# themattrosen/Planeverb

Measured on AMD Instinct MI355X. Metric: grid_cell_updates_per_s, higher is better.
Workload: dtype f32

## Files before the change

include/planeverb_amd.h:

```cpp
#ifndef PLANEVERB_AMD_H
#define PLANEVERB_AMD_H

#include <stddef.h>
#include <stdint.h>

#ifdef __cplusplus
extern "C" {
#endif

#if defined(__GNUC__)
#define PVA_EXPORT __attribute__((visibility("default")))
#else
#define PVA_EXPORT
#endif


typedef struct PlaneverbOutput {
    float occlusion;
    float wetGain;
    float rt60;
    float lowpass;
    float directionX;
    float directionY;
    float sourceDirectionX;
// ... 209 lines not shown
#define PVA_SHAPE_CAPSULE 2
#define PVA_SHAPE_WALL_PATH 3
#define PVA_SHAPE_POLYGON 4
PVA_EXPORT int PvAmdHostRoundShapeCoverage(float gridSizeX, float gridSizeY, int gridResolution, int kind, const float* xy,
                                           int n, float radius, uint8_t* cover);

PVA_EXPORT int PvAmdRun(PvAmdSolver* s, float lx, float ly, float lz);
PVA_EXPORT int PvAmdRunAsync(PvAmdSolver* s, float lx, float ly, float lz);
PVA_EXPORT int PvAmdRunAsyncAfter(PvAmdSolver* s, PvAmdSolver* prev, float lx, float ly, float lz);
PVA_EXPORT int PvAmdSync(PvAmdSolver* s);
PVA_EXPORT int PvAmdRunBatch(PvAmdSolver* const* solvers, int n, const float* listenersXYZ, int wait);
PVA_EXPORT float PvAmdClockProbe(int device, float* byMemtimeMHz);
PVA_EXPORT int PvAmdBandwidthProbe(int device, float* gbPerS4);
PVA_EXPORT int PvAmdGetTimings(PvAmdSolver* s, PvAmdTimings* out);
PVA_EXPORT int PvAmdLastRunResidentWindow(PvAmdSolver* s);

PVA_EXPORT int PvAmdSetEmitters(PvAmdSolver* s, const float* xyz, int n);
PVA_EXPORT int PvAmdGetOutput(PvAmdSolver* s, float ex, float ey, float ez, PlaneverbOutput* out);
PVA_EXPORT int PvAmdSetOutputQueries(PvAmdSolver* s, const float* xyz, int n);
PVA_EXPORT int PvAmdGetQueriedOutputs(PvAmdSolver* s, PlaneverbOutput* out, int n);
PVA_EXPORT int PvAmdCopyResults(PvAmdSolver* s, float* res8, float* delay);
PVA_EXPORT int PvAmdCopyResultsBlock(PvAmdSolver* s, int r0, int c0, int nr, int nc, float* res8, float* delay);
PVA_EXPORT int PvAmdGetImpulseResponse(PvAmdSolver* s, int cx, int cy, float* out3T);
PVA_EXPORT int PvAmdGetImpulseResponseCells(PvAmdSolver* s, int cx, int cy, PlaneverbCell* outT);
PVA_EXPORT int PvAmdCopyFields(PvAmdSolver* s, float* pr, float* vx, float* vy);
PVA_EXPORT int PvAmdCopyHistoryPlane(PvAmdSolver* s, int t, float* pr);
typedef struct PvAmdRoomMetrics {
    float c50, c80, d50, ts, e50, l50, e80, l80, total, moment;
} PvAmdRoomMetrics;
PVA_EXPORT int PvAmdComputeRoomMetrics(PvAmdSolver* s, float* ms);
// ... 62 lines not shown
```

planeverb_amd/api.py:

```python
import ctypes as C
import os
from collections import namedtuple

import numpy as np

from .build import LIB_PATH

PV_INVALID_DRY_GAIN = -1.0
PV_INVALID_ID = -1

PVA_OPT_DENSE_HISTORY = 1
PVA_OPT_NUM_STEPS = 2
PVA_OPT_SKIP_ANALYSIS = 3
PVA_OPT_USE_GRAPH = 4
PVA_OPT_STEPS_PER_LAUNCH = 5
PVA_OPT_TILE_ROWS = 6
PVA_OPT_NO_FREE_GRID = 7
PVA_OPT_TIME_KERNELS = 8
PVA_OPT_TILE_ORDER = 9
PVA_OPT_SMALL_GRID_KERNEL = 10
PVA_OPT_PACKED_MATH = 11
PVA_OPT_STREAMING_ANALYSIS = 12
PVA_OPT_STREAM_ROWS = 13
PVA_OPT_MERGED_LAUNCH = 14
# ... 169 lines not shown
    "PvAmdHostEdgeLayerTablesR0": (C.c_int, [C.c_float, C.c_float, C.c_int, C.POINTER(C.c_int), C.c_double, _fp]),
    "PvAmdHostEdgeLayerTables": (C.c_int, [C.c_float, C.c_float, C.c_int, C.POINTER(C.c_int), _fp]),
    "PvAmdHostEnclosure": (C.c_int, [C.POINTER(C.c_ubyte)] + [C.c_int] * 7 + [C.POINTER(C.c_int)]),
    "PvAmdHostOrientedBoxVertices": (C.c_int, [C.c_float] * 6 + [_fp]),
    "PvAmdHostShape": (C.c_int, [_fp, C.c_int, C.c_float, _fp]),
    "PvAmdHostShapeCoverage": (C.c_int, [C.c_float, C.c_float, C.c_int, _fp, C.c_int, C.POINTER(C.c_ubyte)]),
    "PvAmdHostRoundShapeCoverage": (C.c_int, [C.c_float, C.c_float, C.c_int, C.c_int, _fp, C.c_int, C.c_float,
                                              C.POINTER(C.c_ubyte)]),
    "PvAmdRun": (C.c_int, [_vp] + [C.c_float] * 3),
    "PvAmdRunAsync": (C.c_int, [_vp] + [C.c_float] * 3),
    "PvAmdRunAsyncAfter": (C.c_int, [_vp, _vp] + [C.c_float] * 3),
    "PvAmdSync": (C.c_int, [_vp]),
    "PvAmdRunBatch": (C.c_int, [C.POINTER(_vp), C.c_int, _fp, C.c_int]),
    "PvAmdGetTimings": (C.c_int, [_vp, C.POINTER(PvAmdTimings)]),
    "PvAmdLastRunResidentWindow": (C.c_int, [_vp]),
    "PvAmdClockProbe": (C.c_float, [C.c_int, _fp]),
    "PvAmdBandwidthProbe": (C.c_int, [C.c_int, _fp]),
    "PvAmdSetEmitters": (C.c_int, [_vp, _fp, C.c_int]),
    "PvAmdGetOutput": (C.c_int, [_vp] + [C.c_float] * 3 + [C.POINTER(PlaneverbOutput)]),
    "PvAmdSetOutputQueries": (C.c_int, [_vp, _fp, C.c_int]),
    "PvAmdGetQueriedOutputs": (C.c_int, [_vp, C.POINTER(PlaneverbOutput), C.c_int]),
    "PvAmdCopyResults": (C.c_int, [_vp, _fp, _fp]),
    "PvAmdCopyResultsBlock": (C.c_int, [_vp, C.c_int, C.c_int, C.c_int, C.c_int, _fp, _fp]),
    "PvAmdGetImpulseResponse": (C.c_int, [_vp, C.c_int, C.c_int, _fp]),
    "PvAmdGetImpulseResponseCells": (C.c_int, [_vp, C.c_int, C.c_int, C.POINTER(PlaneverbCell)]),
    "PvAmdCopyFields": (C.c_int, [_vp, _fp, _fp, _fp]),
    "PvAmdCopyHistoryPlane": (C.c_int, [_vp, C.c_int, _fp]),
    "PvAmdComputeRoomMetrics": (C.c_int, [_vp, _fp]),
    "PvAmdCopyRoomMetrics": (C.c_int, [_vp, _fp]),
    "PvAmdCopyRoomMetricsBlock": (C.c_int, [_vp, C.c_int, C.c_int, C.c_int, C.c_int, _fp]),
# ... 847 lines not shown
    def run_async_after(self, prev, listener):
        _check(lib().PvAmdRunAsyncAfter(self._h, prev._h, *[float(v) for v in listener]))

    def sync(self):
        _check(lib().PvAmdSync(self._h))

    def run_steps(self, nsteps, with_pulse=False, listener=(0.0, 0.0, 0.0)):
        _check(lib().PvAmdRunSteps(self._h, int(nsteps), int(with_pulse), float(listener[0]), float(listener[2])))

    def last_run_resident_window(self):
        rc = lib().PvAmdLastRunResidentWindow(self._h)
        if rc < 0:
            raise PlaneverbError(last_error())
        return rc == 1

    def timings(self):
        t = PvAmdTimings()
        _check(lib().PvAmdGetTimings(self._h, t))
        return t

    def set_emitters(self, emitters):
        e = np.ascontiguousarray(emitters, np.float32).reshape(-1, 3)
        _check(lib().PvAmdSetEmitters(self._h, _f(e), len(e)))

    def get_output(self, emitter):
        o = PlaneverbOutput()
        _check(lib().PvAmdGetOutput(self._h, *[float(v) for v in emitter], o))
        return o

    def set_output_queries(self, emitters):
# ... 87 lines not shown
```

planeverb_amd/csrc/pv_analysis.hip:

```cpp
#include <hip/hip_runtime.h>

#include <cfloat>
#include <climits>
#include <cstdint>

#include "pv_analysis.h"
#include "pv_analysis_dev.h"
#include "pv_device.h"
#include "pv_launch.h"
#include "pv_libm.h"
#include "pv_prims.h"
namespace pva {



template <int CH>
__device__ __forceinline__ void rt60Chunk(const float (&pc)[CH], const int i0, const int startingPoint, float& edc,
                                          float& xysum, float& ysum) {
    float e[CH], y[CH];
#pragma unroll
    for (int k = 0; k < CH; ++k) {
        edc = (i0 - k >= startingPoint) ? edc + pc[k] * pc[k] : edc;
        e[k] = edc;
    }
// ... 15 lines not shown
    return *X < a.gx && *Y < a.gy;
}

#ifndef PV_ONSET_WAVES
#define PV_ONSET_WAVES 4
#endif
#ifndef PV_ONSET_SC
#define PV_ONSET_SC 32
#endif
constexpr int kOnsetWaves = PV_ONSET_WAVES, kOnsetSC = PV_ONSET_SC;
__global__ __launch_bounds__(64 * kOnsetWaves) void pv_onset_kernel(const AnalyzeArgs a) {
    __shared__ int found[64];
    if (analysisAborted(a)) return;
    const DynParams dyn = *a.dyn;
    const int lane = threadIdx.x & 63, wave = __builtin_amdgcn_readfirstlane((int)(threadIdx.x >> 6));
    const long long g = (long long)blockIdx.x * 64 + lane;
    const PlaneCell c = planeCell(a, dyn, g);
    const int T = a.T;
    int tF = INT_MAX;
    bool live = c.inGrid;
    if (live) {
        tF = a.tileFirst[c.tile];
        live = tF < T && a.coef[(size_t)(c.X + a.G) * a.pitch + (c.Y + a.G)].beta != 0.f;
    }
    const bool air = live;
    if (a.labels) {
        const int lX = dyn.lrow - a.G, lY = dyn.lcol - a.G;
        const int mine = live ? a.labels[(size_t)c.X * a.labelNY + c.Y] : -1;
        const int theirs = (lX >= 0 && lX <= a.gx && lY >= 0 && lY < a.labelNY) ? a.labels[(size_t)lX * a.labelNY + lY] : -2;
        live = live && mine == theirs;
    }
    if (wave == 0) found[lane] = INT_MAX;
    if (a.stamp && blockIdx.x == 0 && threadIdx.x == 0) a.stamp[1] = wall_clock64();
    __syncthreads();
    bool inPrev = false;
    if (a.box) {
        const int p0 = a.prevBox[0], p1 = a.prevBox[1], p2 = min(a.prevBox[2], a.gx - 1), p3 = min(a.prevBox[3], a.gy - 1);
        inPrev = c.inGrid && c.X >= p0 && c.X <= p2 && c.Y >= p1 && c.Y <= p3;
        if (p2 >= p0 && p3 >= p1) {
            const int wr0 = dyn.histRow0 - a.G, wc0 = dyn.histCol0 - a.G;
            const int wr1 = wr0 + min(a.winRows, a.gx - wr0) - 1, wc1 = wc0 + min(a.winCols, a.gy - wc0) - 1;
            if (p0 < wr0 || p2 > wr1 || p1 < wc0 || p3 > wc1)
                for (int r = p0 + (int)blockIdx.x; r <= p2; r += (int)gridDim.x)
                    for (int cc = p1 + (int)threadIdx.x; cc <= p3; cc += (int)blockDim.x)
                        if (r < wr0 || r > wr1 || cc < wc0 || cc > wc1) a.delay[r * a.gy + cc] = FLT_MAX;
        }
    }
    if (a.wholeWindow || a.box) {
        if (wave == 0 && c.inGrid && !live && (a.wholeWindow || inPrev)) a.delay[c.X * a.gy + c.Y] = FLT_MAX;
        if (blockIdx.x == 0 && wave == 1) {
            int n = 0;
            for (int i = lane; i < dyn.histTilesX * dyn.histTilesY; i += 64) {
                const int ti = dyn.histTileX0 + i / dyn.histTilesY, tj = dyn.histTileY0 + i % dyn.histTilesY;
                if (a.tileFirst[ti * a.nty + tj] < T) n += a.rxi * a.wi;
            }
#pragma unroll
            for (int off = 1; off < 64; off <<= 1) n += __shfl_xor(n, off);
            if (lane == 0) a.activeCount[0] = n;
        }
    }
    if (__ballot(live) == 0ull) {
        const unsigned long long ms = __ballot(air);
        if (wave == 0 && lane == 0 && ms) atomicAdd(a.activeCount + 3, __popcll(ms));
        return;
    }
// ... 42 lines not shown
        }
        if (lane == 0) {
            const int b0 = __hip_atomic_load(a.box + 0, __ATOMIC_RELAXED, __HIP_MEMORY_SCOPE_AGENT);
            const int b1 = __hip_atomic_load(a.box + 1, __ATOMIC_RELAXED, __HIP_MEMORY_SCOPE_AGENT);
            const int b2 = __hip_atomic_load(a.box + 2, __ATOMIC_RELAXED, __HIP_MEMORY_SCOPE_AGENT);
            const int b3 = __hip_atomic_load(a.box + 3, __ATOMIC_RELAXED, __HIP_MEMORY_SCOPE_AGENT);
            if (r0 < b0) atomicMin(a.box + 0, r0);
            if (c0 < b1) atomicMin(a.box + 1, c0);
            if (r1 > b2) atomicMax(a.box + 2, r1);
            if (c1 > b3) atomicMax(a.box + 3, c1);
        }
    }
    if (lane == 0) {
        if (mr) {
            atomicAdd(a.activeCount + 1, __popcll(mr));
            a.unitList[atomicAdd(a.activeCount + 4, 1)] = (int)blockIdx.x;
        }
        if (ms) atomicAdd(a.activeCount + 3, __popcll(ms));
    }
}

__global__ __launch_bounds__(256) void pv_encode_kernel(const AnalyzeArgs a) {
    if (analysisAborted(a)) return;
    const DynParams dyn = *a.dyn;
    const int unit = blockIdx.x * 4 + (int)(threadIdx.x >> 6);
    if (unit >= a.activeCount[4]) return;
    const PlaneCell pc0 = planeCell(a, dyn, (long long)a.unitList[unit] * 64 + (threadIdx.x & 63));
    const float delay = pc0.inGrid ? a.delay[pc0.X * a.gy + pc0.Y] : FLT_MAX;
    const bool live = delay != FLT_MAX;
    if (__ballot(live) == 0ull) return;
    encodeWave<false>(a, dyn, pc0, live, live ? (int)delay : 0, rt60LanesPerCell(a, a.activeCount[1]) == 1);
// ... 155 lines not shown
    for (int i = 0; i < dirJumpPasses(a.T); ++i) hipLaunchKernelGGL(pv_dir_jump_kernel, grid, block, 0, stream, a, J);
    hipLaunchKernelGGL(pv_dir_final_kernel, grid, block, 0, stream, a, J);
}

__global__ void pv_fill_delay_kernel(float* delay, int n) {
    const int i = blockIdx.x * blockDim.x + threadIdx.x;
    if (i < n) delay[i] = FLT_MAX;
}

void launchFarCells(const AnalyzeArgs& a, hipStream_t stream) {
    const int n = a.gx * a.gy;
    hipLaunchKernelGGL(pv_far_cells_kernel, dim3((n + 255) / 256), dim3(256), 0, stream, a);
}

void launchOnset(const AnalyzeArgs& a, hipStream_t stream) {
    hipLaunchKernelGGL(pv_onset_kernel, dim3((unsigned)((a.histPlane + 63) / 64)), dim3(64 * kOnsetWaves), 0, stream, a);
}
void launchEncode(const AnalyzeArgs& a, hipStream_t stream) {
    const unsigned units = (unsigned)((a.histPlane + 63) / 64);
    if (a.rt60Lanes != 1 && a.histPlane <= 16384)
        hipLaunchKernelGGL(pv_encode_groups_kernel<16>, dim3(units * 4), dim3(256), 0, stream, a);
    else if (a.rt60Lanes != 1 && a.histPlane <= kRt60TileMinCells)
        hipLaunchKernelGGL(pv_encode_groups_kernel<4>, dim3(units), dim3(256), 0, stream, a);
    else
        hipLaunchKernelGGL(pv_encode_kernel, dim3((unsigned)((a.histPlane + 255) / 256)), dim3(256), 0, stream, a);
}
void launchRt60(const AnalyzeArgs& a, hipStream_t stream) { launchRt60Forms(a, stream); }

void launchAnalysisCells(const AnalyzeArgs& a, hipStream_t stream) {
    launchOnset(a, stream);
    launchEncode(a, stream);
// ... 240 lines not shown
```

planeverb_amd/csrc/pv_capi.cpp:

```cpp
#include <algorithm>
#include <climits>
#include <cstdio>
#include <cstring>
#include <memory>
#include <new>
#include <string>

#include "../../include/planeverb_amd.h"
#include "pv_context.h"
#include "pv_core.h"
#include "pv_metrics.h"
#ifndef PVA_HOST_TEST
#include "pv_bake.h"
#include "pv_shard.h"
#include "pv_slabs.h"
#include "pv_launch.h"
#include "pv_layer.h"
#include "pv_solver.h"
#endif

using namespace pva;

static thread_local std::string g_lastError;

// ... 947 lines not shown
    out->generalKernelMs = t.generalKernelMs;
    out->airLaunches = t.airLaunches;
    out->generalLaunches = t.generalLaunches;
    out->stepLoopMs = t.stepLoopMs;
    out->reachedCells = t.reachedCells;
    out->activeCells = t.activeCells;
    out->silentCells = t.silentCells;
    return 0;
} PV_API_CATCH(-1)

int PvAmdLastRunResidentWindow(PvAmdSolver* h) try {
    if (!wholeGrid(h) || !ensure(h, true)) return -1;
    return h->s->lastRunResidentWindow() ? 1 : 0;
} PV_API_CATCH(-1)

int PvAmdSetEmitters(PvAmdSolver* h, const float* xyz, int n) try {
    if (!wholeGrid(h) || !ensure(h) || (n > 0 && !xyz)) return -1;
    return ret(h, h->s->setEmitters(xyz, n));
} PV_API_CATCH(-1)

int PvAmdGetOutput(PvAmdSolver* h, float ex, float ey, float ez, PlaneverbOutput* out) try {
    if (!wholeGrid(h) || !out || !ensure(h, true)) return -1;
    float v[8];
    bool valid = false;
    if (!(h->g ? h->g->getOutput(ex, ey, ez, v, &valid) : h->s->getOutput(ex, ey, ez, v, &valid))) return ret(h, false);
    if (!valid) {
        std::memset(out, 0, sizeof(*out));
        out->occlusion = kInvalidDryGain;
        return 0;
    }
// ... 529 lines not shown
```

planeverb_amd/csrc/pv_device.h:

```cpp
#pragma once

#include <hip/hip_runtime.h>

#include <cstdint>

namespace pva {

constexpr float kCDev = 343.21f;
constexpr float kAudibleThresholdDev = 0.00000316f;
constexpr float kDistanceGainDev = 0.891251f;
constexpr float kDelayCloseDev = 5.f;

struct FaceCoef {
    float kx, ky, beta;
};
constexpr uint32_t kAirFaceBits = 0x7fc00000u;

struct Geometry {
    int gx, gy, NX, NY;
    int G;
    int rxi, wi;
    int ntx, nty;
    int rows, pitch;
    int x0, NXg, gxg;
// ... 132 lines not shown
    int xcdTarget;
    long long histPlane;
    long long planeBytes;
    int pitch, G;
    int ntx, nty, ntiles;
    int T;
    float courant;
    unsigned long long* stamp;
    int histSub;
    int winTi0, winTj0;
    int gridNty;
    int winRow0, winCol0;
    int window;
};

struct HaloHandoff {
    unsigned* count;
    unsigned* raise[2];
    const unsigned* await[2];
    unsigned seq;
    int* err;
    unsigned* abortWord;
};

struct OpenArgs {
    int* sOnset;
    float* sEdry;
    float* sFx;
    float* sFy;
    uint8_t* cellsOpen2;
// ... 34 lines not shown
struct AnalyzeArgs {
    const unsigned* abortWord;
    const float* hist;
    const FaceCoef* coef;
    const int* tileFirst;
    const DynParams* dyn;
    float* out;
    float* delay;
    long long resN;
    long long histPlane;
    int histPitch;
    int pitch, G;
    int gx, gy;
    int rxi, wi, nty;
    int winRows, winCols;
    int* activeCount;
    int* unitList;
    int* dirScratch;
    int dirJump;
    int rt60Lanes;
    int rt60Tile;
    int T;
    int nDir, nDry, nWet, nCut;
    unsigned fs;
    int res;
    float dx;
    float courant;
    float efree;
    float lx, lz;
    int lcx, lcy;
// ... 39 lines not shown
```

planeverb_amd/csrc/pv_fused.hip:

```cpp
#include <hip/hip_runtime.h>

#include <cfloat>
#include <climits>
#include <cstdint>
#include <cstdlib>

#include "pv_analysis.h"
#include "pv_analysis_dev.h"
#include "pv_device.h"
#include "pv_launch.h"
#include "pv_libm.h"
#include "pv_prims.h"

namespace pva {

#ifdef PV_EXPERIMENTAL
namespace {

constexpr int kFusedThreads = 320;
constexpr int kFusedOnsetSC = 8;
constexpr unsigned kFusedSpinLimit = 1u << 20;

struct FusedShared {
    double tab[96];
// ... 237 lines not shown
    unsigned grid = (unsigned)std::min<long long>(std::max<long long>(items, 64), 1024);
    if (const char* e = std::getenv("PLANEVERB_AMD_FUSED_WORKERS"))
        if (std::atoi(e) > 0) grid = std::min(grid, (unsigned)std::atoi(e));
    hipLaunchKernelGGL(pv_analysis_fused_kernel, dim3(grid), dim3(kFusedThreads), 0, stream, f);
}
#else
bool fusedAnalysisBuilt() { return false; }
bool fusedAnalysisOk(const AnalyzeArgs&) { return false; }
void launchAnalysisFused(const FusedArgs&, hipStream_t) {}
#endif

namespace {
__global__ __launch_bounds__(512) void pv_run_finish_kernel(const float* __restrict__ res, long long n, const long long* cells, int nq,
                                                            float* out, const FarInfo f, int* err, int* counts,
                                                            const unsigned* claims, int* status, unsigned* zeroWords, int nZero,
                                                            unsigned long long* stamp) {
    if (stamp && threadIdx.x == 0) stamp[2] = wall_clock64();
    const int q = threadIdx.x >> 3, k = threadIdx.x & 7;
    if (q < nq) {
        const long long c = cells[q];
        float v = c >= 0 ? res[k * n + c] : 0.f;
        if (c >= 0 && (k == 4 || k == 5) && isFarCell(f, c)) {
            float x, y;
            farDirectionOf(f, c, &x, &y);
            v = k == 4 ? x : y;
        }
        out[q * 8 + k] = v;
    }
    const int claimed = claims ? (int)*claims : -1;
    __syncthreads();
    for (int i = threadIdx.x; i < nZero; i += 512) zeroWords[i] = 0u;
    if (threadIdx.x == 0) {
        status[0] = *err;
        if (nZero > 0) *err = 0;
        status[1] = counts[0];
        status[2] = counts[1];
        status[3] = claimed;
        status[4] = counts[3];
        counts[1] = 0;
        counts[2] = 0;
        counts[3] = 0;
        counts[4] = 0;
    }
}
}

void launchRunFinish(const float* res, long long n, const long long* cellsHost, int nq, float* outHost, const FarInfo& far,
                     int* err, int* counts, const unsigned* claims, int* statusHost, unsigned* zeroWords, int nZero,
                     unsigned long long* stamp, hipStream_t stream) {
    hipLaunchKernelGGL(pv_run_finish_kernel, dim3(1), dim3(512), 0, stream, res, n, cellsHost, nq, outHost, far, err, counts, claims,
                       statusHost, zeroWords, nZero, stamp);
}

}
```

planeverb_amd/csrc/pv_launch.h:

```cpp
#pragma once

#include <hip/hip_runtime.h>

#include <cstdint>

#include "pv_device.h"

namespace pva {

bool stepConfigSupported(int K, int rxi);
bool mergedConfigOk(int K, int rxi);
bool stepConfigStacked(int K, int rxi);
int stepConfigExtraRows(int K, int rxi);
void launchStep(int K, int rxi, const StepArgs& a, hipStream_t stream, int which = 3, hipStream_t stream2 = nullptr);
constexpr int kStepGeneralPacked = 32;
bool patchConfigOk(int K, int rxi);
void launchStepPatch(int K, int rxi, const StepArgs& a, int blocks, hipStream_t stream);
bool openConfigOk(int K, int rxi);
bool unpackedAirOk();
void launchStreamClassify(const ClassifyArgs& c, hipStream_t stream);
void launchStreamIdle(const ClassifyArgs& c, int* idleHost, hipStream_t stream);
void launchStepOpen(int K, int rxi, const StepArgs& a, const OpenArgs& o, hipStream_t stream);
int segConfigColumns(int K, int rxi);
int segConfigMaxTileColumns(int K, int rxi);
// ... 40 lines not shown
void launchAnalysisDirection(const AnalyzeArgs& a, hipStream_t stream);
void launchFarDirections(float* res, long long n, const FarInfo& far, hipStream_t stream);
void launchFillDelay(float* delay, long long n, hipStream_t stream);
void launchStreamAccum(const AnalyzeArgs& a, const uint8_t* hasEmitter, uint8_t* tileOpen, int ntiles,
                       hipStream_t stream);
void launchStreamFinalize(const AnalyzeArgs& a, hipStream_t stream);

void launchCarryResults(const AnalyzeArgs& a, const float* srcOut, int srcR0, int srcC0, int srcNR, int srcNC, hipStream_t stream);
void launchRt60Forms(const AnalyzeArgs& a, hipStream_t stream);

bool fusedAnalysisBuilt();
bool fusedAnalysisOk(const AnalyzeArgs& a);
void launchAnalysisFused(const FusedArgs& f, hipStream_t stream);
void launchRunFinish(const float* res, long long n, const long long* cellsHost, int nq, float* outHost, const FarInfo& far,
                     int* err, int* counts, const unsigned* claims, int* statusHost, unsigned* zeroWords, int nZero,
                     unsigned long long* stamp, hipStream_t stream);

void launchRoomMetrics(const AnalyzeArgs& a, float* out, hipStream_t stream);

void launchHaloPush(const float* const src[6], float* const dst[6], long long n, const HaloHandoff& hand, hipStream_t stream);
void launchHistRow(const AnalyzeArgs& a, int X, float* outTxPitch, hipStream_t stream);
void launchCopyBlock(const float* src, long long sstride, int spitch, int sr0, int sc0, float* dst, long long dstride,
                     int dpitch, int dr0, int dc0, int nr, int nc, int nplanes, const int* srcPlanesDev,
                     const int* dstPlanesDev, hipStream_t stream, const unsigned* abortWord = nullptr);
void launchGatherQueries(const float* res, long long n, const long long* cellsHost, int nq, float* outHost, const FarInfo& far,
                         hipStream_t stream);
void launchGatherOutput(const float* res, long long n, long long cell, float* out8Host, const FarInfo& far, hipStream_t stream);
void launchPackResults(const float* res, long long n, float* res8, hipStream_t stream);
void launchPackWindow(const float* res, long long n, int gy, int r0, int c0, int nr, int nc, float* out8, const FarInfo& far,
                      hipStream_t stream);
void launchEfree(const float* hist, long long plane, long long cellOff, int n, float r, float* out,
// ... 9 lines not shown
```

planeverb_amd/csrc/pv_solver.cpp:

```cpp
#include "pv_solver.h"
#include "pv_boundary.h"
#include "pv_layer.h"
#include "pv_shapes.h"

#include <unistd.h>

#include <algorithm>
#include <atomic>
#include <chrono>
#include <climits>
#include <cmath>
#include <cstdlib>
#include <cstring>
#include <limits>
#include <memory>
#include <mutex>

#include "pv_launch.h"
#include "pv_metrics.h"

namespace pva {

#ifndef PV_LABEL_MAX_CELLS
#define PV_LABEL_MAX_CELLS (1100 * 1100)
// ... 453 lines not shown
                      kGuard >= K_ + residentExtraRows(K_, rxi_) && T_ >= 1;
        if (useResident) {
            const int cap = residentMaxBlocks(K_, rxi_, device_);
            residentBudget_ = cap * 3 / 4;
            if (ntiles > std::min(residentBudget_, kResidentMaxTiles)) useResident = false;
        }
        resFlagWords_ = useResident ? ntiles + 2 : 0;
        bool& windowOk = caps_.windowOk;
        windowOk = opt_.residentWindow != 0 && !useResident && K_ == 12 && rxi_ == 36 && residentConfigOk(K_, 12) &&
                    wi_ == 64 - 2 * K_ && kGuard >= K_ + residentExtraRows(K_, 12) && !opt_.streaming && !isSlab() && T_ >= 1;
        if (windowOk) {
            residentBudget_ = residentMaxBlocks(K_, 12, device_) * 3 / 4;
            resFlagWords_ = std::min(residentBudget_, kResidentMaxTiles) + 2;
            if (residentBudget_ < 3) windowOk = false;
        }
        if (resFlagWords_ > 0 && !dalloc(&resFlags_, (size_t)resFlagWords_, true)) return false;
        if (useResident) {
            static std::atomic<int> turn{0};
            xcdTarget_ = turn.fetch_add(1) & 7;
            if (const char* e = std::getenv("PLANEVERB_AMD_RESIDENT_XCD_TARGET")) xcdTarget_ = std::atoi(e);
            if (const char* e = std::getenv("PLANEVERB_AMD_RESIDENT_XCD")) {
                xcdOk_ = std::atoi(e) != 0;
                if (std::atoi(e) > 1) kResidentXcdMaxTiles = std::min(std::atoi(e), 128);
            }
        }
    }

    {
        const bool wanted = opt_.fusedAnalysis > 0;
        if (wanted && !fusedAnalysisBuilt())
// ... 62 lines not shown
    for (float* p : sState_)
        if (p) hipFree(p);
    if (sOnset_) hipFree(sOnset_);
    if (tileOpen_) hipFree(tileOpen_);
    if (tileMarks_) hipFree(tileMarks_);
    if (tileEmit_) hipFree(tileEmit_);
    for (void* p : {(void*)classStream_, (void*)ringOpen_, (void*)cellsOpen2_, (void*)openList_, (void*)openCount_, (void*)ringList_})
        if (p) hipFree(p);
    if (ringHost_) hipHostFree(ringHost_);
    if (idleHost_) hipHostFree(idleHost_);
    releaseResident();
#ifdef PV_RESIDENT_TRACE
    if (caps_.useResident) residentDumpTrace();
#endif
    if (resFlags_) hipFree(resFlags_);
    if (metrics_) hipFree(metrics_);
    for (auto& e : metricsEv_)
        if (e) hipEventDestroy(e);
    if (layerList_) hipFree(layerList_);
    if (layerTab_) hipFree(layerTab_);
    if (px_[0]) hipFree(px_[0]);
    if (emCells_) hipFree(emCells_);
    if (emTrace_) hipFree(emTrace_);
    void* ptrs[] = {coef_,      matDev_, pulseDev_, hist_,  tileFirst_, tileClass_, generalList_,
                    generalCount_, dynDev_, errFlag_, res8_,     delay_, scratch_, res_, activeCount_, win8_, unitList_, fusedCtl_, labelDev_, nearBox_,
                    histAbove_, histEdge_, tileDead_, deadCount_, matBaseDev_, shapeDev_};
    for (void* p : ptrs)
        if (p) hipFree(p);
    for (size_t b = 1; b < bandStream_.size(); ++b)
        if (bandStream_[b]) {
// ... 454 lines not shown
    {
        const char* e = getenv("PLANEVERB_AMD_GENERAL_PACKED");
        const long long nt = (long long)geo_.ntx * geo_.nty;
        stepWhich_ = 4 | (((e ? atoi(e) != 0 : (long long)count * 100 >= 8 * nt)) ? kStepGeneralPacked : 0);
    }
    if (airChanged) {
        enclosures_.clear();
        windowOff_ = false;
    }
    if ((airChanged || !labelsValid_) && !makeLabels()) return false;
    mat_.clearDirty();
    geometryDirty_ = false;
    boundaryDirty_ = false;
    layerDirty_ = false;
    planesDirty_ = true;
    dynValid_ = false;
    dropGraph();
    tim_.geometryMs =
        std::chrono::duration<float, std::milli>(std::chrono::steady_clock::now() - t0).count();
    return true;
}

bool Solver::makeLabels() {
    const size_t n = (size_t)g_.NX * g_.NY;
    if (isSlab() || opt_.streaming || opt_.skipAnalysis || n > (size_t)PV_LABEL_MAX_CELLS) return labelsValid_ = true;
    if (!labelDev_ && !dalloc(&labelDev_, n, false)) return false;
    labelHost_.assign(n, -1);
    std::vector<int> stack;
    int next = 0;
    const int NX = g_.NX, NY = g_.NY;
// ... 311 lines not shown
    if (!e || !e->found) return false;
    const DynParams& d = dynCur_;
    if (e->ti0 < d.histTileX0 || e->ti0 + e->tis > d.histTileX0 + d.histTilesX || e->tj0 < d.histTileY0 ||
        e->tj0 + e->tjs > d.histTileY0 + d.histTilesY || e->ti0 + e->tis > geo_.ntx || e->tj0 + e->tjs > geo_.nty)
        return false;
    const int blocks = 3 * e->tis * e->tjs;
    if (blocks > std::min(residentBudget_, kResidentMaxTiles)) return false;
    if (!reserveBlocks(residentInFlight(device_), blocks, residentBudget_, &residentHeld_)) return false;
    win[0] = e->ti0;
    win[1] = e->tis;
    win[2] = e->tj0;
    win[3] = e->tjs;
    return true;
}

void Solver::enqueueWindowRun(const int win[4]) {
    enqueueBeginRun(true);
    launchResidentRun(12, win);
    for (int i = 0; i < 4; ++i) reachRect_[i] = win[i];
}

void Solver::launchResidentRun(int tileRows, const int* win) {
    if (stampTimed()) stampsHost_[0] = stampsHost_[1] = stampsHost_[2] = 0ull;
    launchResident(K_, tileRows, residentArgs(win), stream_);
    tim_.stepLaunches = ceilDiv(T_, K_);
    cur_ = tim_.stepLaunches & 1;
}

ResidentArgs Solver::residentArgs(const int* win) const {
    const long long off = win ? (long long)win[0] * rxi_ * geo_.pitch + (long long)win[2] * wi_ : 0;
    ResidentArgs ra{};
    for (int i = 0; i < 2; ++i) {
        ra.pr[i] = pr_[i] + off;
        ra.vx[i] = vx_[i] + off;
// ... 274 lines not shown
    a.resN = (long long)std::max(lgx_, 1) * g_.gy;
    a.delay = delay_;
    a.histPlane = histPlane_;
    a.histPitch = histPitch_;
    a.pitch = geo_.pitch;
    a.G = geo_.G;
    a.gx = lgx_;
    a.gy = g_.gy;
    a.x0 = x0_;
    a.histAbove = histAbove_;
    a.rxi = rxi_;
    a.wi = wi_;
    a.nty = geo_.nty;
    a.winRows = histTilesX_ * rxi_;
    a.winCols = histTilesY_ * wi_;
    a.activeCount = activeCount_;
    a.unitList = unitList_;
    a.dirScratch = reinterpret_cast<int*>(scratch_);
    const bool smallWindow = a.winRows <= 256 && a.winCols <= 256;
    a.dirJump = (!opt_.denseHistory && !(smallWindow && geo_.ntx * geo_.nty > 4096)) ? 1 : 0;
    a.rt60Lanes = (opt_.rt60Lanes == 16 || opt_.rt60Lanes == 4 || opt_.rt60Lanes == 1) ? opt_.rt60Lanes : 0;
    a.rt60Tile = (a.rt60Lanes == 1 || (a.rt60Lanes == 0 && histPlane_ > kRt60TileMinCells &&
                                       (lastReached_ < 0 || lastReached_ > kRt60TileMinCells / 2))) ? 1 : 0;
    a.T = T_;
    a.nDir = g_.nDir;
    a.nDry = g_.nDry;
    a.nWet = g_.nWet;
    a.nCut = g_.nCut;
    a.fs = g_.fs;
    a.res = g_.res;
// ... 106 lines not shown
    launchAnalysisDirection(a, stream_);
    if (fork) hipStreamWaitEvent(stream_, anaEv_[1], 0);
    if (lazyFar_) {
        farWin_ = curWindow();
        farDirValid_ = false;
    }
    if (a.box) nearPar_ ^= 1;
    nearBoxValid_ = a.box != nullptr;
}

bool Solver::beginRun(PathRun::Kind kind, int lcx, int lcy, bool withPulse, float lx, float lz) {
    if (pendingTimings_ && !sync()) return false;
    metricsValid_ = false;
    lastRun_ = LastRun::Failed;
    if (!applyGeometry()) return false;
    PathRun r;
    r.kind = kind;
    r.listenerInside = withPulse && lcx >= 0 && lcx <= g_.gx && lcy >= 0 && lcy <= g_.gy;
    r.layerActive = layerActive();
    r.layerTiles = numLayer_ > 0;
    r.windowOff = windowOff_;
    plan_ = planRun(caps_, r);
    if (!prepareDyn(lcx, lcy, withPulse)) return false;
    if (plan_.segments && numSeg_ == 0) {
        r.segmentsFound = false;
        plan_ = planRun(caps_, r);
    }
    tim_.stepLaunches = 0;
    kevUsed_ = 0;
    launchCap_ = numGeneral_;
    if (kind == PathRun::Raw) {
        planesDirty_ = true;
        return true;
    }
    if (!zeroPlanesIfNeeded()) return false;
    lastLx_ = lx;
    lastLz_ = lz;
    cur_ = 0;
    if (plan_.reach) return clearReachPlanes();
    sweptDirty_ = true;
    return true;
}

bool Solver::enqueueRun(int lcx, int lcy, float lx, float lz) {
    const auto inUse = queue_.lockUse();
    if (!hipOk(hipSetDevice(device_), "hipSetDevice")) return false;
    if (!beginRun(PathRun::Run, lcx, lcy, true, lx, lz)) return false;
    if (plan_.path == StepPath::Streaming) return enqueueStreamingRun(lx, lz);
    lastLcx_ = lcx;
    lastLcy_ = lcy;
    releaseResident();
    int win[4] = {0, 0, 0, 0};
    if (plan_.path == StepPath::Window && !windowFor(lcx, lcy, win)) plan_.path = plan_.fallback;
    if (plan_.path == StepPath::Resident && !reserveBlocks(residentInFlight(device_), caps_.ntiles, residentBudget_, &residentHeld_))
        plan_.path = plan_.fallback;
    if (!stampTimed()) hipEventRecord(ev_[0], stream_);
    switch (plan_.path) {
        case StepPath::Window: enqueueWindowRun(win); break;
        case StepPath::Resident: enqueueResidentRun(); break;
        case StepPath::SmallGrid:
            if (!enqueueSmallGridRun()) return false;
            break;
        case StepPath::Graph:
            if (!enqueueGraphRun()) return false;
            break;
        case StepPath::Launches:
            if (!enqueueResetAndSteps()) return false;
            break;
        case StepPath::Streaming: break;
    }
    if (!stampTimed()) hipEventRecord(ev_[1], stream_);
    if (!opt_.skipAnalysis) enqueueAnalysis(lx, lz);
    if (!stampTimed()) hipEventRecord(ev_[2], stream_);
    lastRunBatched_ = false;
    launchRunFinish(res_, (long long)g_.gx * g_.gy, qCellsHost_, opt_.skipAnalysis ? 0 : numQueries_, qOutHost_, farInfo(), errFlag_,
                    activeCount_, plan_.oneXcd ? resFlags_ + geo_.ntx * geo_.nty + 1 : nullptr, statusHost_, resFlags_,
                    resFlags_ ? resFlagWords_ : 0, stampTimed() ? stampsHost_ : nullptr, stream_);
    if (stampTimed()) hipEventRecord(ev_[2], stream_);
    enqueueTap();
    statusQueued_ = true;
    pendingTimings_ = true;
    return hipOk(hipGetLastError(), "run launch");
}

bool Solver::enqueueStreamingRun(float lx, float lz) {
    const int ntiles = geo_.ntx * geo_.nty;
    hipEventRecord(ev_[0], stream_);
    const size_t nres = (size_t)g_.gx * g_.gy;
    if (!hipOk(hipMemsetAsync(sOnset_, 0xff, nres * 4, stream_), "state reset")) return false;
    for (float* p : sState_)
        if (!hipOk(hipMemsetAsync(p, 0, nres * 4, stream_), "state reset")) return false;
    if (numEmitters_ > 0 &&
// ... 317 lines not shown
        if (statusQueued_) {
            statusQueued_ = false;
            flag = statusHost_[0];
            counts[0] = statusHost_[1];
            counts[1] = statusHost_[2];
            tim_.silentCells = statusHost_[4];
            if (plan_.oneXcd && statusHost_[3] >= 0 && statusHost_[3] < geo_.ntx * geo_.nty && flag == 0) flag = 4;
        } else {
            hipStream_t fs = lastRunBatched_ ? stream2_ : stream_;
            if (!hipOk(hipMemcpyAsync(&flag, errFlag_, sizeof(int), hipMemcpyDeviceToHost, fs), "errFlag copy") ||
                !hipOk(hipMemcpyAsync(counts, activeCount_, sizeof(counts), hipMemcpyDeviceToHost, fs), "count copy") ||
                !hipOk(hipStreamSynchronize(fs), "errFlag sync"))
                return false;
            if (flag) hipMemsetAsync(errFlag_, 0, sizeof(int), fs);
        }
        tim_.reachedCells = counts[1];
        lastReached_ = counts[1];
        tim_.activeCells = counts[0];
        const struct {
            int flag;
            bool applies;
            bool* form;
            bool value;
            const char* message;
        } giveUps[] = {
            {4, xcdOk_, &xcdOk_, false,
             "[planeverb_amd] resident kernel: one-XCD mode not available on this device (workgroups are "
             "not spread over the XCDs as expected); using the placement-independent hand-off\n"},
            {3, plan_.path == StepPath::Window, &windowOff_, true,
             "[planeverb_amd] resident window: a workgroup gave up waiting for its neighbours (the device is "
// ... 255 lines not shown
bool Solver::copyFields(float* pr, float* vx, float* vy) {
    if (!hipOk(hipSetDevice(device_), "hipSetDevice")) return false;
    const size_t n = (size_t)lNX_ * g_.NY;
    const float* src[3] = {pr_[cur_], vx_[cur_], vy_[cur_]};
    float* dst[3] = {pr, vx, vy};
    for (int i = 0; i < 3; ++i) {
        if (!dst[i]) continue;
        launchUnpad(src[i], scratch_, geo_, stream_);
        if (!hipOk(hipMemcpyAsync(dst[i], scratch_, n * 4, hipMemcpyDeviceToHost, stream_), "field copy")) return false;
        if (!hipOk(hipStreamSynchronize(stream_), "field sync")) return false;
    }
    return true;
}

bool Solver::setFields(const float* pr, const float* vx, const float* vy) {
    if (isSlab()) return fail("setFields is not available on a slab");
    planesDirty_ = true;
    if (!hipOk(hipSetDevice(device_), "hipSetDevice")) return false;
    const size_t n = (size_t)g_.NX * g_.NY;
    const float* src[3] = {pr, vx, vy};
    float* dst[3] = {pr_[cur_], vx_[cur_], vy_[cur_]};
    const size_t planeBytes = (size_t)geo_.rows * geo_.pitch * 4;
    for (float* p : px_)
        if (p && !hipOk(hipMemsetAsync(p, 0, planeBytes, stream_), "field clear")) return false;
    for (int i = 0; i < 3; ++i) {
        if (!hipOk(hipMemsetAsync(dst[i], 0, planeBytes, stream_), "field clear")) return false;
        if (!src[i]) continue;
        if (!hipOk(hipMemcpyAsync(scratch_, src[i], n * 4, hipMemcpyHostToDevice, stream_), "field upload")) return false;
        launchPad(scratch_, dst[i], geo_, stream_);
        if (!hipOk(hipStreamSynchronize(stream_), "field sync")) return false;
// ... 103 lines not shown
```

planeverb_amd/csrc/pv_solver.h:

```cpp
#pragma once

#include <hip/hip_runtime.h>

#include <cstdint>
#include <memory>
#include <mutex>
#include <string>
#include <vector>

#include "pv_core.h"
#include "pv_device.h"

namespace pva {

struct SolverOptions {
    int K = 0;
    int rxi = 0;
    bool denseHistory = false;
    int numSteps = 0;
    bool skipAnalysis = false;
    int useGraph = 0;
    bool withFreeGrid = true;
    int tileOrder = -1;
    int merged = 1;
// ... 68 lines not shown

    const GridSpec& spec() const { return g_; }
    const Geometry& geometry() const { return geo_; }
    int device() const { return device_; }
    int K() const { return K_; }
    int rxi() const { return rxi_; }
    float efree() const { return efree_; }
    void setEfree(float e) { efree_ = e; }
    int T() const { return T_; }
    long long deviceBytes() const { return deviceBytes_; }
    int histRows() const { return histRows_; }
    int histPitch() const { return histPitch_; }
    const std::string& lastError() const { return err_; }
    bool streamFuse() const { return streamFuse_; }
    bool lastRunResidentWindow() const { return plan_.path == StepPath::Window; }
    bool residentKernel() const { return caps_.useResident && !layerActive(); }
    SolverOptions& options() { return opt_; }

    int addBox(const Box& b);
    bool updateBox(int id, const Box& b);
    bool removeBox(int id);
    int numBoxes() const;
    std::vector<std::pair<int, Box>> boxes() const;
    void rasterAdd(const Box& b) {
        mat_.add(b);
        metricsValid_ = false;
    }
    void rasterRemove(const Box& b) {
        mat_.remove(b);
        metricsValid_ = false;
// ... 204 lines not shown
    int numRing_ = 0;
    std::vector<uint8_t> emTilesHost_;
    int* openCount_ = nullptr;
    int* emCells_ = nullptr;
    float* emTrace_ = nullptr;
    int numEmitters_ = 0, emCap_ = 0;
    unsigned* resFlags_ = nullptr;
    int residentHeld_ = 0;
    bool xcdOk_ = true;
    int xcdTarget_ = 0;
    int xcdHeld_ = 0;
    int lastLcx_ = 0, lastLcy_ = 0;
    void releaseResident();
    bool windowOff_ = false;
    int resFlagWords_ = 0;
    struct EnclosureRec {
        Enclosure e;
        std::vector<int> cells;
    };
    std::vector<EnclosureRec> enclosures_;
    const Enclosure* enclosureOf(int lcx, int lcy);
    bool windowFor(int lcx, int lcy, int win[4]);
    ResidentArgs residentArgs(const int* win) const;
    void enqueueWindowRun(const int win[4]);
    float* scratch_ = nullptr;
    float* metrics_ = nullptr;
    bool metricsValid_ = false;
    DynParams metricsDyn_{};
    std::vector<float> metricsHost_;
    bool metricsHostValid_ = false;
    hipEvent_t metricsEv_[2] = {nullptr, nullptr};
    enum class LastRun { None, Failed, Ok };
    LastRun lastRun_ = LastRun::None;
    bool fetchRoomMetrics();
    size_t scratchCount_ = 0;

    DynParams* dynHost_ = nullptr;
    float* outHost_ = nullptr;
    int* statusHost_ = nullptr;
// ... 81 lines not shown
```

Baseline: 36990 billion.

## Chain back-to-back window runs and restrict onset analysis to the run window

When consecutive runs use the resident window path, the solver now skips the begin-run reset and plane clearing. It double-buffers the per-tile first-arrival table, and the finish kernel resets the spare table for the previous window. The onset analysis kernel is launched over a 2D grid covering only the window's tile rectangle instead of the whole history plane. This cuts per-run clearing and analysis work, at the cost of added state-tracking complexity and a risk of stale data if the chain invalidation misses a case.

Result: faster. 38350 billion (median of 6 runs) (+3.7%).

```diff
diff --git a/include/planeverb_amd.h b/include/planeverb_amd.h
--- a/include/planeverb_amd.h
+++ b/include/planeverb_amd.h
@@ -247,6 +247,7 @@
 PVA_EXPORT int PvAmdBandwidthProbe(int device, float* gbPerS4);
 PVA_EXPORT int PvAmdGetTimings(PvAmdSolver* s, PvAmdTimings* out);
 PVA_EXPORT int PvAmdLastRunResidentWindow(PvAmdSolver* s);
+PVA_EXPORT int PvAmdLastRunOneXcd(PvAmdSolver* s);
 
 PVA_EXPORT int PvAmdSetEmitters(PvAmdSolver* s, const float* xyz, int n);
 PVA_EXPORT int PvAmdGetOutput(PvAmdSolver* s, float ex, float ey, float ez, PlaneverbOutput* out);
diff --git a/planeverb_amd/api.py b/planeverb_amd/api.py
--- a/planeverb_amd/api.py
+++ b/planeverb_amd/api.py
@@ -207,6 +207,7 @@
     "PvAmdRunBatch": (C.c_int, [C.POINTER(_vp), C.c_int, _fp, C.c_int]),
     "PvAmdGetTimings": (C.c_int, [_vp, C.POINTER(PvAmdTimings)]),
     "PvAmdLastRunResidentWindow": (C.c_int, [_vp]),
+    "PvAmdLastRunOneXcd": (C.c_int, [_vp]),
     "PvAmdClockProbe": (C.c_float, [C.c_int, _fp]),
     "PvAmdBandwidthProbe": (C.c_int, [C.c_int, _fp]),
     "PvAmdSetEmitters": (C.c_int, [_vp, _fp, C.c_int]),
@@ -1084,6 +1085,12 @@
             raise PlaneverbError(last_error())
         return rc == 1
 
+    def last_run_one_xcd(self):
+        rc = lib().PvAmdLastRunOneXcd(self._h)
+        if rc < 0:
+            raise PlaneverbError(last_error())
+        return rc == 1
+
     def timings(self):
         t = PvAmdTimings()
         _check(lib().PvAmdGetTimings(self._h, t))
diff --git a/planeverb_amd/csrc/pv_analysis.hip b/planeverb_amd/csrc/pv_analysis.hip
--- a/planeverb_amd/csrc/pv_analysis.hip
+++ b/planeverb_amd/csrc/pv_analysis.hip
@@ -53,7 +53,16 @@
     if (analysisAborted(a)) return;
     const DynParams dyn = *a.dyn;
     const int lane = threadIdx.x & 63, wave = __builtin_amdgcn_readfirstlane((int)(threadIdx.x >> 6));
-    const long long g = (long long)blockIdx.x * 64 + lane;
+    long long grp = blockIdx.x;
+    const int bid = (int)(blockIdx.y * gridDim.x + blockIdx.x), nblk = (int)(gridDim.x * gridDim.y);
+    if (a.onsetTis > 0) {
+        const long long tileCells = (long long)a.rxi * a.wi, rowCells = (long long)dyn.histTilesY * tileCells;
+        const long long beg = (long long)(a.onsetTi0 - dyn.histTileX0 + (int)blockIdx.y) * rowCells + (long long)(a.onsetTj0 - dyn.histTileY0) * tileCells;
+        const long long end = beg + (long long)a.onsetTjs * tileCells;
+        grp = beg / 64 + blockIdx.x;
+        if (grp * 64 >= end || (blockIdx.y > 0 && grp * 64 < end - rowCells)) grp = (a.histPlane + 63) / 64;
+    }
+    const long long g = grp * 64 + lane;
     const PlaneCell c = planeCell(a, dyn, g);
     const int T = a.T;
     int tF = INT_MAX;
@@ -70,24 +79,28 @@
         live = live && mine == theirs;
     }
     if (wave == 0) found[lane] = INT_MAX;
-    if (a.stamp && blockIdx.x == 0 && threadIdx.x == 0) a.stamp[1] = wall_clock64();
+    if (a.stamp && bid == 0 && threadIdx.x == 0) a.stamp[1] = wall_clock64();
     __syncthreads();
     bool inPrev = false;
     if (a.box) {
         const int p0 = a.prevBox[0], p1 = a.prevBox[1], p2 = min(a.prevBox[2], a.gx - 1), p3 = min(a.prevBox[3], a.gy - 1);
         inPrev = c.inGrid && c.X >= p0 && c.X <= p2 && c.Y >= p1 && c.Y <= p3;
         if (p2 >= p0 && p3 >= p1) {
-            const int wr0 = dyn.histRow0 - a.G, wc0 = dyn.histCol0 - a.G;
-            const int wr1 = wr0 + min(a.winRows, a.gx - wr0) - 1, wc1 = wc0 + min(a.winCols, a.gy - wc0) - 1;
+            int wr0 = dyn.histRow0 - a.G, wc0 = dyn.histCol0 - a.G;
+            int wr1 = wr0 + min(a.winRows, a.gx - wr0) - 1, wc1 = wc0 + min(a.winCols, a.gy - wc0) - 1;
+            if (a.onsetTis > 0) {
+                wr0 = a.onsetTi0 * a.rxi, wc0 = a.onsetTj0 * a.wi;
+                wr1 = min(wr0 + a.onsetTis * a.rxi, a.gx) - 1, wc1 = min(wc0 + a.onsetTjs * a.wi, a.gy) - 1;
+            }
             if (p0 < wr0 || p2 > wr1 || p1 < wc0 || p3 > wc1)
-                for (int r = p0 + (int)blockIdx.x; r <= p2; r += (int)gridDim.x)
+                for (int r = p0 + bid; r <= p2; r += nblk)
                     for (int cc = p1 + (int)threadIdx.x; cc <= p3; cc += (int)blockDim.x)
                         if (r < wr0 || r > wr1 || cc < wc0 || cc > wc1) a.delay[r * a.gy + cc] = FLT_MAX;
         }
     }
     if (a.wholeWindow || a.box) {
         if (wave == 0 && c.inGrid && !live && (a.wholeWindow || inPrev)) a.delay[c.X * a.gy + c.Y] = FLT_MAX;
-        if (blockIdx.x == 0 && wave == 1) {
+        if (bid == 0 && wave == 1) {
             int n = 0;
             for (int i = lane; i < dyn.histTilesX * dyn.histTilesY; i += 64) {
                 const int ti = dyn.histTileX0 + i / dyn.histTilesY, tj = dyn.histTileY0 + i % dyn.histTilesY;
@@ -160,7 +173,7 @@
     if (lane == 0) {
         if (mr) {
             atomicAdd(a.activeCount + 1, __popcll(mr));
-            a.unitList[atomicAdd(a.activeCount + 4, 1)] = (int)blockIdx.x;
+            a.unitList[atomicAdd(a.activeCount + 4, 1)] = (int)grp;
         }
         if (ms) atomicAdd(a.activeCount + 3, __popcll(ms));
     }
@@ -346,7 +359,9 @@
 }
 
 void launchOnset(const AnalyzeArgs& a, hipStream_t stream) {
-    hipLaunchKernelGGL(pv_onset_kernel, dim3((unsigned)((a.histPlane + 63) / 64)), dim3(64 * kOnsetWaves), 0, stream, a);
+    const dim3 grid = a.onsetTis > 0 ? dim3((unsigned)(((long long)a.onsetTjs * a.rxi * a.wi + 63) / 64 + 1), (unsigned)a.onsetTis)
+                                     : dim3((unsigned)((a.histPlane + 63) / 64));
+    hipLaunchKernelGGL(pv_onset_kernel, grid, dim3(64 * kOnsetWaves), 0, stream, a);
 }
 void launchEncode(const AnalyzeArgs& a, hipStream_t stream) {
     const unsigned units = (unsigned)((a.histPlane + 63) / 64);
diff --git a/planeverb_amd/csrc/pv_capi.cpp b/planeverb_amd/csrc/pv_capi.cpp
--- a/planeverb_amd/csrc/pv_capi.cpp
+++ b/planeverb_amd/csrc/pv_capi.cpp
@@ -985,6 +985,11 @@
     return h->s->lastRunResidentWindow() ? 1 : 0;
 } PV_API_CATCH(-1)
 
+int PvAmdLastRunOneXcd(PvAmdSolver* h) try {
+    if (!wholeGrid(h) || !ensure(h, true)) return -1;
+    return h->s->lastRunOneXcd() ? 1 : 0;
+} PV_API_CATCH(-1)
+
 int PvAmdSetEmitters(PvAmdSolver* h, const float* xyz, int n) try {
     if (!wholeGrid(h) || !ensure(h) || (n > 0 && !xyz)) return -1;
     return ret(h, h->s->setEmitters(xyz, n));
diff --git a/planeverb_amd/csrc/pv_device.h b/planeverb_amd/csrc/pv_device.h
--- a/planeverb_amd/csrc/pv_device.h
+++ b/planeverb_amd/csrc/pv_device.h
@@ -170,6 +170,12 @@
     int window;
 };
 
+struct FirstReset {
+    int* table;
+    int nty;
+    int ti0, tis, tj0, tjs;
+};
+
 struct HaloHandoff {
     unsigned* count;
     unsigned* raise[2];
@@ -234,6 +240,7 @@
     int gx, gy;
     int rxi, wi, nty;
     int winRows, winCols;
+    int onsetTi0, onsetTis, onsetTj0, onsetTjs;
     int* activeCount;
     int* unitList;
     int* dirScratch;
diff --git a/planeverb_amd/csrc/pv_fused.hip b/planeverb_amd/csrc/pv_fused.hip
--- a/planeverb_amd/csrc/pv_fused.hip
+++ b/planeverb_amd/csrc/pv_fused.hip
@@ -275,7 +275,7 @@
 __global__ __launch_bounds__(512) void pv_run_finish_kernel(const float* __restrict__ res, long long n, const long long* cells, int nq,
                                                             float* out, const FarInfo f, int* err, int* counts,
                                                             const unsigned* claims, int* status, unsigned* zeroWords, int nZero,
-                                                            unsigned long long* stamp) {
+                                                            unsigned long long* stamp, const FirstReset fr) {
     if (stamp && threadIdx.x == 0) stamp[2] = wall_clock64();
     const int q = threadIdx.x >> 3, k = threadIdx.x & 7;
     if (q < nq) {
@@ -291,6 +291,8 @@
     const int claimed = claims ? (int)*claims : -1;
     __syncthreads();
     for (int i = threadIdx.x; i < nZero; i += 512) zeroWords[i] = 0u;
+    if (fr.table)
+        for (int i = threadIdx.x; i < fr.tis * fr.tjs; i += 512) fr.table[(fr.ti0 + i / fr.tjs) * fr.nty + fr.tj0 + i % fr.tjs] = INT_MAX;
     if (threadIdx.x == 0) {
         status[0] = *err;
         if (nZero > 0) *err = 0;
@@ -308,9 +310,9 @@
 
 void launchRunFinish(const float* res, long long n, const long long* cellsHost, int nq, float* outHost, const FarInfo& far,
                      int* err, int* counts, const unsigned* claims, int* statusHost, unsigned* zeroWords, int nZero,
-                     unsigned long long* stamp, hipStream_t stream) {
+                     unsigned long long* stamp, const FirstReset& firstReset, hipStream_t stream) {
     hipLaunchKernelGGL(pv_run_finish_kernel, dim3(1), dim3(512), 0, stream, res, n, cellsHost, nq, outHost, far, err, counts, claims,
-                       statusHost, zeroWords, nZero, stamp);
-}
-
-}
+                       statusHost, zeroWords, nZero, stamp, firstReset);
+}
+
+}
diff --git a/planeverb_amd/csrc/pv_launch.h b/planeverb_amd/csrc/pv_launch.h
--- a/planeverb_amd/csrc/pv_launch.h
+++ b/planeverb_amd/csrc/pv_launch.h
@@ -78,7 +78,7 @@
 void launchAnalysisFused(const FusedArgs& f, hipStream_t stream);
 void launchRunFinish(const float* res, long long n, const long long* cellsHost, int nq, float* outHost, const FarInfo& far,
                      int* err, int* counts, const unsigned* claims, int* statusHost, unsigned* zeroWords, int nZero,
-                     unsigned long long* stamp, hipStream_t stream);
+                     unsigned long long* stamp, const FirstReset& firstReset, hipStream_t stream);
 
 void launchRoomMetrics(const AnalyzeArgs& a, float* out, hipStream_t stream);
 
diff --git a/planeverb_amd/csrc/pv_solver.cpp b/planeverb_amd/csrc/pv_solver.cpp
--- a/planeverb_amd/csrc/pv_solver.cpp
+++ b/planeverb_amd/csrc/pv_solver.cpp
@@ -491,6 +491,9 @@
             resFlagWords_ = std::min(residentBudget_, kResidentMaxTiles) + 2;
             if (residentBudget_ < 3) windowOk = false;
         }
+        if (windowOk && (!dalloc(&tileFirstSpare_, (size_t)ntiles, false) ||
+                         !hipOk(hipMemsetD32Async((hipDeviceptr_t)tileFirstSpare_, INT_MAX, (size_t)ntiles, stream_), "tileFirst")))
+            return false;
         if (resFlagWords_ > 0 && !dalloc(&resFlags_, (size_t)resFlagWords_, true)) return false;
         if (useResident) {
             static std::atomic<int> turn{0};
@@ -583,6 +586,7 @@
     if (caps_.useResident) residentDumpTrace();
 #endif
     if (resFlags_) hipFree(resFlags_);
+    if (tileFirstSpare_) hipFree(tileFirstSpare_);
     if (metrics_) hipFree(metrics_);
     for (auto& e : metricsEv_)
         if (e) hipEventDestroy(e);
@@ -1067,6 +1071,7 @@
     boundaryDirty_ = false;
     layerDirty_ = false;
     planesDirty_ = true;
+    windowChain_ = false;
     dynValid_ = false;
     dropGraph();
     tim_.geometryMs =
@@ -1408,10 +1413,21 @@
     return true;
 }
 
-void Solver::enqueueWindowRun(const int win[4]) {
-    enqueueBeginRun(true);
+bool Solver::enqueueWindowRun(const int win[4]) {
+    const bool sameWindow = win[0] == reachRect_[0] && win[1] == reachRect_[1] && win[2] == reachRect_[2] && win[3] == reachRect_[3];
+    chained_ = chainIn_ && !opt_.denseHistory;
+    if (!(chained_ && sameWindow && T_ > K_ && !planesDirty_ && !sweptDirty_) && !clearReachPlanes()) return false;
+    if (chained_) {
+        std::swap(tileFirst_, tileFirstSpare_);
+        dropGraph();
+        for (int i = 0; i < 4; ++i) spareWin_[i] = runWin_[i];
+    } else {
+        enqueueBeginRun(true);
+    }
+    for (int i = 0; i < 4; ++i) runWin_[i] = win[i];
     launchResidentRun(12, win);
     for (int i = 0; i < 4; ++i) reachRect_[i] = win[i];
+    return true;
 }
 
 void Solver::launchResidentRun(int tileRows, const int* win) {
@@ -1716,6 +1732,12 @@
     a.nty = geo_.nty;
     a.winRows = histTilesX_ * rxi_;
     a.winCols = histTilesY_ * wi_;
+    if (plan_.path == StepPath::Window) {
+        a.onsetTi0 = runWin_[0];
+        a.onsetTis = runWin_[1];
+        a.onsetTj0 = runWin_[2];
+        a.onsetTjs = runWin_[3];
+    }
     a.activeCount = activeCount_;
     a.unitList = unitList_;
     a.dirScratch = reinterpret_cast<int*>(scratch_);
@@ -1852,6 +1874,9 @@
     metricsValid_ = false;
     lastRun_ = LastRun::Failed;
     if (!applyGeometry()) return false;
+    chainIn_ = windowChain_;
+    windowChain_ = false;
+    chained_ = false;
     PathRun r;
     r.kind = kind;
     r.listenerInside = withPulse && lcx >= 0 && lcx <= g_.gx && lcy >= 0 && lcy <= g_.gy;
@@ -1875,7 +1900,7 @@
     lastLx_ = lx;
     lastLz_ = lz;
     cur_ = 0;
-    if (plan_.reach) return clearReachPlanes();
+    if (plan_.reach) return (kind == PathRun::Run && plan_.path == StepPath::Window) ? true : clearReachPlanes();
     sweptDirty_ = true;
     return true;
 }
@@ -1889,12 +1914,17 @@
     lastLcy_ = lcy;
     releaseResident();
     int win[4] = {0, 0, 0, 0};
-    if (plan_.path == StepPath::Window && !windowFor(lcx, lcy, win)) plan_.path = plan_.fallback;
+    if (plan_.path == StepPath::Window && !windowFor(lcx, lcy, win)) {
+        plan_.path = plan_.fallback;
+        if (!clearReachPlanes()) return false;
+    }
     if (plan_.path == StepPath::Resident && !reserveBlocks(residentInFlight(device_), caps_.ntiles, residentBudget_, &residentHeld_))
         plan_.path = plan_.fallback;
     if (!stampTimed()) hipEventRecord(ev_[0], stream_);
     switch (plan_.path) {
-        case StepPath::Window: enqueueWindowRun(win); break;
+        case StepPath::Window:
+            if (!enqueueWindowRun(win)) return false;
+            break;
         case StepPath::Resident: enqueueResidentRun(); break;
         case StepPath::SmallGrid:
             if (!enqueueSmallGridRun()) return false;
@@ -1911,9 +1941,12 @@
     if (!opt_.skipAnalysis) enqueueAnalysis(lx, lz);
     if (!stampTimed()) hipEventRecord(ev_[2], stream_);
     lastRunBatched_ = false;
+    FirstReset fr{};
+    if (chained_) fr = FirstReset{tileFirstSpare_, geo_.nty, spareWin_[0], spareWin_[1], spareWin_[2], spareWin_[3]};
     launchRunFinish(res_, (long long)g_.gx * g_.gy, qCellsHost_, opt_.skipAnalysis ? 0 : numQueries_, qOutHost_, farInfo(), errFlag_,
                     activeCount_, plan_.oneXcd ? resFlags_ + geo_.ntx * geo_.nty + 1 : nullptr, statusHost_, resFlags_,
-                    resFlags_ ? resFlagWords_ : 0, stampTimed() ? stampsHost_ : nullptr, stream_);
+                    resFlags_ ? resFlagWords_ : 0, stampTimed() ? stampsHost_ : nullptr, fr, stream_);
+    windowChain_ = plan_.path == StepPath::Window;
     if (stampTimed()) hipEventRecord(ev_[2], stream_);
     enqueueTap();
     statusQueued_ = true;
@@ -2261,6 +2294,7 @@
                 return false;
             if (flag) hipMemsetAsync(errFlag_, 0, sizeof(int), fs);
         }
+        if (flag) windowChain_ = false;
         tim_.reachedCells = counts[1];
         lastReached_ = counts[1];
         tim_.activeCells = counts[0];
@@ -2546,6 +2580,7 @@
 }
 
 bool Solver::setFields(const float* pr, const float* vx, const float* vy) {
+    windowChain_ = false;
     if (isSlab()) return fail("setFields is not available on a slab");
     planesDirty_ = true;
     if (!hipOk(hipSetDevice(device_), "hipSetDevice")) return false;
diff --git a/planeverb_amd/csrc/pv_solver.h b/planeverb_amd/csrc/pv_solver.h
--- a/planeverb_amd/csrc/pv_solver.h
+++ b/planeverb_amd/csrc/pv_solver.h
@@ -106,6 +106,7 @@
     const std::string& lastError() const { return err_; }
     bool streamFuse() const { return streamFuse_; }
     bool lastRunResidentWindow() const { return plan_.path == StepPath::Window; }
+    bool lastRunOneXcd() const { return plan_.path == StepPath::Resident && plan_.oneXcd; }
     bool residentKernel() const { return caps_.useResident && !layerActive(); }
     SolverOptions& options() { return opt_; }
 
@@ -340,6 +341,11 @@
     void releaseResident();
     bool windowOff_ = false;
     int resFlagWords_ = 0;
+    int* tileFirstSpare_ = nullptr;
+    int spareWin_[4] = {0, 0, 0, 0};
+    bool windowChain_ = false, chainIn_ = false;
+    bool chained_ = false;
+    int runWin_[4] = {0, 0, 0, 0};
     struct EnclosureRec {
         Enclosure e;
         std::vector<int> cells;
@@ -348,7 +354,7 @@
     const Enclosure* enclosureOf(int lcx, int lcy);
     bool windowFor(int lcx, int lcy, int win[4]);
     ResidentArgs residentArgs(const int* win) const;
-    void enqueueWindowRun(const int win[4]);
+    bool enqueueWindowRun(const int win[4]);
     float* scratch_ = nullptr;
     float* metrics_ = nullptr;
     bool metricsValid_ = false;
```
